# Advaith-Sajeev/LiDAR-Vision-VQA

Hardware: AMD Instinct MI355X
Metric: fused tokens/sec/GPU + cross-attn MFMA-roofline % (32k pts x 196 patches) (higher is better)
Workload: dtype bf16; 1 GPU; BASELINE configs[1]: 32768-pt scenes (Dist-C) -> hard voxelise (0.1, 0.1, 0.2) T=10 max=60000 + MeanVFE; pillars (0.2, 0.2, 8.0) T=20 max=30000 -> PillarVFE[64] -> PointPillarScatter 512x512 (as an index map; sparse key stream: K|V computed only for the cells with a pillar in their 3x3 neighbourhood, by LayerNorm and the K|V projection folded onto the 64-channel conv token, every other key from th; parallelism=scene-parallel x1

## Files before the change

### lidar-vision-vqa_amd/csrc/bev_tiles.hip

```cpp
#include "common.h"
#include <type_traits>
#include <utility>

namespace bt {

typedef __attribute__((ext_vector_type(8))) short bf16x8;
typedef __attribute__((ext_vector_type(4))) float f32x4;
typedef __attribute__((ext_vector_type(2))) __bf16 bf16x2_t;
typedef uint32_t u32x4 __attribute__((ext_vector_type(4)));

__device__ __forceinline__ uint32_t pack_bf16(float a, float b) {
    bf16x2_t p = {(__bf16)a, (__bf16)b};
    return *reinterpret_cast<uint32_t *>(&p);
}
typedef _Float16 f16x2_t __attribute__((ext_vector_type(2)));
__device__ __forceinline__ uint32_t pack_f16(float a, float b) {
    f16x2_t p = {(_Float16)a, (_Float16)b};
    return __builtin_bit_cast(uint32_t, p);
}

constexpr int TS = 8, TCELLS = 64;
constexpr int NPIECE = 8, PCELLS = 8;
constexpr int PH = 4, PW = 6, PHALO = PH * PW;
constexpr int NSLOT = NPIECE * PHALO;
// ... 832 lines not shown
    __syncthreads();
    if (g_begin >= g_end) return;
    {
        int c0, c1;
        const int i0 = load_idx(g_begin, c0);
        const int i1 = g_begin + g_step < g_end ? load_idx(g_begin + g_step, c1) : (c1 = -1, -1);
        store_idx(idxh, i0, c0);
        store_idx(idxh + 256, i1, c1);
    }
    __syncthreads();
    dma_halo(idxh);
    asm volatile("s_waitcnt vmcnt(0)" ::: "memory");
    __syncthreads();
    conv_tile(idxh, 0);
    int buf = 0;
    for (int64_t g = g_begin, it = 0; g < g_end; g += g_step, ++it) {
        __syncthreads();
        const int32_t *ih_cur = idxh + (it & 1) * 256, *ih_nx = idxh + ((it + 1) & 1) * 256;
        const bool has_nx = g + g_step < g_end, has_n2 = g + 2 * g_step < g_end;
        if (has_nx) dma_halo(ih_nx);
        int code_cur[4];
#pragma unroll
        for (int gq = 0; gq < 4; ++gq) code_cur[gq] = ih_cur[200 + 2 * gq + (l15 >> 3)];
        int c2 = -1;
        const int i2 = has_n2 ? load_idx(g + 2 * g_step, c2) : -1;
        {
            const int rt = wid & 3;
            const uint16_t *rp = r_hi + (16 * rt + l15) * C + 8 * g4, *rpl = r_lo + (16 * rt + l15) * C + 8 * g4;
            const bf16x8 ra0 = *reinterpret_cast<const bf16x8 *>(rp), ra1 = *reinterpret_cast<const bf16x8 *>(rp + 32);
            bf16x8 rl0 = ra0, rl1 = ra1;
            if (X3) { rl0 = *reinterpret_cast<const bf16x8 *>(rpl); rl1 = *reinterpret_cast<const bf16x8 *>(rpl + 32); }
            const f32x4 rinit = *reinterpret_cast<const f32x4 *>(r0s + 16 * rt + 4 * g4);
#pragma unroll
            for (int u = 0; u < 2; ++u) {
                const int gq = 2 * (wid >> 2) + u;
                bf16x8 th0, th1, tl0, tl1;
                load_t(buf, gq, th0, th1, tl0, tl1);
                f32x4 v = rinit;
                v = __builtin_amdgcn_mfma_f32_16x16x32_bf16(ra0, th0, v, 0, 0, 0);
                v = __builtin_amdgcn_mfma_f32_16x16x32_bf16(ra1, th1, v, 0, 0, 0);
                if (X3) {
                    v = __builtin_amdgcn_mfma_f32_16x16x32_bf16(ra0, tl0, v, 0, 0, 0);
                    v = __builtin_amdgcn_mfma_f32_16x16x32_bf16(ra1, tl1, v, 0, 0, 0);
                    v = __builtin_amdgcn_mfma_f32_16x16x32_bf16(rl0, th0, v, 0, 0, 0);
                    v = __builtin_amdgcn_mfma_f32_16x16x32_bf16(rl1, th1, v, 0, 0, 0);
                }
                float sq = (v[0] * v[0] + v[1] * v[1]) + (v[2] * v[2] + v[3] * v[3]);
                sq += __shfl_xor(sq, 16);
                sq += __shfl_xor(sq, 32);
                if (g4 == 0) part[(buf * 4 + rt) * TCELLS + gq * 16 + l15] = sq;
            }
        }
        asm volatile("s_waitcnt vmcnt(0)" ::: "memory");
        __syncthreads();
        store_idx(idxh + (it & 1) * 256, i2, c2);
        {
            const float *pr = part + buf * 4 * TCELLS;
            auto cell_of = [&](int gq) { return gq * 16 + l15; };
            auto code_of = [&](int gq) { return gq == 0 ? code_cur[0] : gq == 1 ? code_cur[1] : gq == 2 ? code_cur[2] : code_cur[3]; };
            auto request = [&](int gq, f32x4 (&te)[2 * JH], int2 &pd) {
                const int cell = cell_of(gq), code = code_of(gq);
                const bool in_list = code >= 0;
                const int64_t prow = in_list ? (int64_t)((code >> 3) / a.S) * TCELLS + (code & 7) * PCELLS + (cell & 7) : 0;
                pd = in_list ? a.piece_dirty[g * NPIECE + (cell >> 3)] : make_int2(0, 0);
                const float *tep = a.te + prow * (2 * N) + ncol0 + col0;
#pragma unroll
                for (int jj = 0; jj < 2 * JH; ++jj) te[jj] = *reinterpret_cast<const f32x4 *>(tep + 4 * jj);
            };
            auto emit = [&](int gq, const f32x4 (&te)[2 * JH], const int2 pd) {
                const int cell = cell_of(gq);
                const bool valid = (pd.y >> (cell & 7)) & 1;
                const int64_t orow = pd.x + __popc((unsigned)pd.y & ((1u << (cell & 7)) - 1u));
                const float ss = (pr[cell] + pr[TCELLS + cell]) + (pr[2 * TCELLS + cell] + pr[3 * TCELLS + cell]) + a.c0;
                const float rstd = 1.0f / sqrtf(ss * a.inv_d + a.eps);
                bf16x8 th0, th1, tl0, tl1;
                load_t(buf, gq, th0, th1, tl0, tl1);
                uint16_t *dst = a.out + orow * (2 * N) + ncol0 + col0;
                auto half_out = [&](auto hf_tag) {
                    constexpr int HF = decltype(hf_tag)::value;
                    f32x4 acc[JH];
                    product(hf_tag, th0, th1, tl0, tl1, acc);
                    uint32_t oh[2 * JH];
#pragma unroll
                    for (int jj = 0; jj < JH; ++jj) {
                        const f32x4 tv = te[HF * JH + jj];
                        oh[2 * jj] = pack_bf16(acc[jj][0] * rstd + tv[0], acc[jj][1] * rstd + tv[1]);
                        oh[2 * jj + 1] = pack_bf16(acc[jj][2] * rstd + tv[2], acc[jj][3] * rstd + tv[3]);
                    }
                    if (valid) {
#pragma unroll
                        for (int q = 0; q < 2 * JH; q += 2)
                            *reinterpret_cast<uint2 *>(dst + 2 * (2 * HF * JH + q)) = make_uint2(oh[q], oh[q + 1]);
                    }
                };
                half_out(std::integral_constant<int, 0>{});
                half_out(std::integral_constant<int, 1>{});
            };
            f32x4 te_a[2 * JH], te_b[2 * JH];
            int2 pd_a, pd_b;
            request(0, te_a, pd_a);
            if (has_nx) conv_tile(ih_nx, buf ^ 1);
            request(1, te_b, pd_b);
            emit(0, te_a, pd_a);
            request(2, te_a, pd_a);
            emit(1, te_b, pd_b);
            request(3, te_b, pd_b);
            emit(2, te_a, pd_a);
            emit(3, te_b, pd_b);
        }
        buf ^= 1;
    }
}

struct ConvArgs {
    const float *feat;
    const int32_t *idx;
    const int32_t *live_list;
    const int2 *piece_dirty;
    const int32_t *counts;
    const float *w9, *b9;
    const uint16_t *rh, *rl;
    const float *r0;
    float c0, inv_d, eps;
    int S, H, W;
    uint16_t *th, *tl;
    float *rstd;
    int32_t *key;
};

typedef int i32x2 __attribute__((ext_vector_type(2)));
template <int N> __device__ __forceinline__ void vm_wait() { asm volatile("s_waitcnt vmcnt(%0)" ::"n"(N) : "memory"); }
template <int OFF> __device__ __forceinline__ void vm_load16(f32x4 &d, const void *p) {
    asm volatile("global_load_dwordx4 %0, %1, off offset:%2" : "=&v"(d) : "v"(p), "n"(OFF) : "memory");
}
__device__ __forceinline__ void vm_load8(i32x2 &d, const void *p) { asm volatile("global_load_dwordx2 %0, %1, off" : "=&v"(d) : "v"(p) : "memory"); }
template <class T> __device__ __forceinline__ void vm_load4(T &d, const void *p) {
    static_assert(sizeof(T) == 4, "one dword");
    asm volatile("global_load_dword %0, %1, off" : "=&v"(d) : "v"(p) : "memory");
}
__device__ __forceinline__ void vm_dma16(const void *src, uint32_t dst) {
    uint32_t keep;
    asm volatile("s_mov_b32 %0, m0\n\ts_mov_b32 m0, %2\n\ts_nop 0\n\tglobal_load_lds_dwordx4 %1, off\n\ts_mov_b32 m0, %0"
                 : "=&s"(keep) : "v"(src), "s"(dst) : "memory");
}
template <class T> __device__ __forceinline__ void landed(T &x) { asm volatile("" : "+v"(x)); }
template <int... I, class F> __device__ __forceinline__ void static_for(std::integer_sequence<int, I...>, F &&f) { (f(std::integral_constant<int, I>{}), ...); }
template <int N, class F> __device__ __forceinline__ void static_for(F &&f) { static_for(std::make_integer_sequence<int, N>{}, f); }
__device__ __forceinline__ void lds_barrier() {
    asm volatile("s_waitcnt lgkmcnt(0)" ::: "memory");
    __builtin_amdgcn_s_barrier();
    asm volatile("" ::: "memory");
}

template <bool X3>
__global__ void __launch_bounds__(512) k_conv_rows(ConvArgs a) {
    constexpr int C = 64, NWV = 8, RING = 8;
    extern __shared__ __attribute__((aligned(16))) uint8_t smem[];
    uint16_t *t_hi = reinterpret_cast<uint16_t *>(smem);
    uint16_t *t_lo = t_hi + TCELLS * C;
    float *halo = reinterpret_cast<float *>(t_lo + TCELLS * C);
    int32_t *idxh = reinterpret_cast<int32_t *>(halo + 2 * NSLOT * C);
    int32_t *mcode = idxh + 2 * 256;
    i32x2 *mdirty = reinterpret_cast<i32x2 *>(mcode + RING * NPIECE);
    float *part = reinterpret_cast<float *>(mdirty + RING * NPIECE);
    const int tid = threadIdx.x, lane = tid & 63, wid = tid >> 6, l15 = lane & 15, g4 = lane >> 4;
    const int tw = a.W / TS;
    const int n_live = a.counts[0];
    const int64_t n_groups = ((int64_t)n_live + NPIECE - 1) / NPIECE;
    const int64_t g_begin = blockIdx.x, g_step = gridDim.x;
    if (g_begin >= n_groups) return;
    const int n_my = (int)((n_groups - g_begin + g_step - 1) / g_step);

    float wk[9][8], bk[8];
#pragma unroll
    for (int c = 0; c < 8; ++c) {
        const int ch = (tid & 7) * 8 + c;
        bk[c] = a.b9 ? a.b9[ch] : 0.f;
#pragma unroll
        for (int k = 0; k < 9; ++k) wk[k][c] = a.w9[ch * 9 + k];
    }
    const int rt = wid & 3;
    bf16x8 ra0, ra1, rl0, rl1;
    {
        const uint16_t *rp = a.rh + (16 * rt + l15) * C + 8 * g4;
        ra0 = *reinterpret_cast<const bf16x8 *>(rp);
        ra1 = *reinterpret_cast<const bf16x8 *>(rp + 32);
        rl0 = ra0; rl1 = ra1;
        if (X3) {
            const uint16_t *rpl = a.rl + (16 * rt + l15) * C + 8 * g4;
            rl0 = *reinterpret_cast<const bf16x8 *>(rpl);
            rl1 = *reinterpret_cast<const bf16x8 *>(rpl + 32);
        }
    }
    f32x4 rinit = *reinterpret_cast<const f32x4 *>(a.r0 + 16 * rt + 4 * g4);

    auto piece_k = [&](int o, int j, bool &ok) -> int64_t {
        const int64_t grp = g_begin + (int64_t)o * g_step, k = grp * NPIECE + j;
        ok = o < n_my && k < n_live;
        return ok ? k : 0;
    };
    auto idx_off = [&](int o, bool &ok) -> int64_t {
        ok = false;
        if (tid >= NSLOT) return 0;
        const int j = tid / PHALO, hc = tid - j * PHALO;
        const int code = mcode[(o & (RING - 1)) * NPIECE + j];
        if (code < 0) return 0;
        const int p = code & 7, ts = code >> 3, t = ts / a.S, sc = ts - t * a.S;
        int y0, x0;
        piece_origin(t, p, tw, y0, x0);
        const int gy = y0 - 1 + hc / PW, gx = x0 - 1 + hc % PW;
        if (gy < 0 || gy >= a.H || gx < 0 || gx >= a.W) return 0;
        ok = true;
        return ((int64_t)sc * a.H + gy) * a.W + gx;
    };
    const uint32_t lds_halo = (uint32_t)(uintptr_t)((__attribute__((address_space(3))) float *)halo);
    auto dma_halo = [&](const int32_t *ih, int hbuf) {
        for (int q = wid; q < NSLOT / 4; q += NWV) {
            const int row = ih[q * 4 + (lane >> 4)];
            const uint32_t dst = __builtin_amdgcn_readfirstlane(lds_halo + (uint32_t)((hbuf * NSLOT + q * 4) * C * 4));
            if (row >= 0) vm_dma16(a.feat + (int64_t)row * C + 4 * l15, dst);
        }
    };
    auto conv_tile = [&](const int32_t *ih, const float *hl, int o) {
        const int cell = tid >> 3, cg = (tid & 7) * 8, hb = (cell >> 3) * PHALO, cy = (cell >> 2) & 1, cx = cell & 3;
        float acc[8];
#pragma unroll
        for (int c = 0; c < 8; ++c) acc[c] = bk[c];
#pragma unroll
        for (int rr = 0; rr < 3; ++rr)
#pragma unroll
            for (int k = 0; k < 3; ++k) {
                const int slot = hb + (cy + rr) * PW + cx + k;
                if (ih[slot] >= 0) {
                    const f32x4 v0 = *reinterpret_cast<const f32x4 *>(hl + slot * C + cg), v1 = *reinterpret_cast<const f32x4 *>(hl + slot * C + cg + 4);
                    const float *kk = wk[rr * 3 + k];
#pragma unroll
                    for (int c = 0; c < 4; ++c) { acc[c] = fmaf(v0[c], kk[c], acc[c]); acc[4 + c] = fmaf(v1[c], kk[4 + c], acc[4 + c]); }
                }
            }
        uint32_t hi[4], lo[4];
#pragma unroll
        for (int c = 0; c < 4; ++c) {
            const float y0 = gelu_erf(acc[2 * c]), y1 = gelu_erf(acc[2 * c + 1]);
            hi[c] = pack_bf16(y0, y1);
            lo[c] = pack_bf16(y0 - __uint_as_float(hi[c] << 16), y1 - __uint_as_float(hi[c] & 0xffff0000u));
        }
        const int ch = (tid & 7) ^ ((cell >> 1) & 7);
        *reinterpret_cast<u32x4 *>(t_hi + cell * C + ch * 8) = u32x4{hi[0], hi[1], hi[2], hi[3]};
        if (X3) *reinterpret_cast<u32x4 *>(t_lo + cell * C + ch * 8) = u32x4{lo[0], lo[1], lo[2], lo[3]};
        const int m = (o & (RING - 1)) * NPIECE + (cell >> 3);
        if (mcode[m] >= 0) {
            const i32x2 pd = mdirty[m];
            if ((pd.y >> (cell & 7)) & 1) {
                const int64_t orow = pd.x + __popc((unsigned)pd.y & ((1u << (cell & 7)) - 1u));
                *reinterpret_cast<u32x4 *>(a.th + orow * C + cg) = u32x4{hi[0], hi[1], hi[2], hi[3]};
                if (X3) *reinterpret_cast<u32x4 *>(a.tl + orow * C + cg) = u32x4{lo[0], lo[1], lo[2], lo[3]};
            }
        }
    };
    auto row_sums = [&]() {
#pragma unroll
        for (int u = 0; u < 2; ++u) {
            const int gq = 2 * (wid >> 2) + u;
            const int row = gq * 16 + l15;
            const int c0 = (g4 ^ ((row >> 1) & 7)) * 8, c1 = ((4 + g4) ^ ((row >> 1) & 7)) * 8;
            const bf16x8 th0 = *reinterpret_cast<const bf16x8 *>(t_hi + row * C + c0), th1 = *reinterpret_cast<const bf16x8 *>(t_hi + row * C + c1);
            f32x4 v = rinit;
            v = __builtin_amdgcn_mfma_f32_16x16x32_bf16(ra0, th0, v, 0, 0, 0);
            v = __builtin_amdgcn_mfma_f32_16x16x32_bf16(ra1, th1, v, 0, 0, 0);
            if (X3) {
                const bf16x8 tl0 = *reinterpret_cast<const bf16x8 *>(t_lo + row * C + c0), tl1 = *reinterpret_cast<const bf16x8 *>(t_lo + row * C + c1);
                v = __builtin_amdgcn_mfma_f32_16x16x32_bf16(ra0, tl0, v, 0, 0, 0);
                v = __builtin_amdgcn_mfma_f32_16x16x32_bf16(ra1, tl1, v, 0, 0, 0);
                v = __builtin_amdgcn_mfma_f32_16x16x32_bf16(rl0, th0, v, 0, 0, 0);
                v = __builtin_amdgcn_mfma_f32_16x16x32_bf16(rl1, th1, v, 0, 0, 0);
            }
            float sq = (v[0] * v[0] + v[1] * v[1]) + (v[2] * v[2] + v[3] * v[3]);
            sq += __shfl_xor(sq, 16);
            sq += __shfl_xor(sq, 32);
            if (g4 == 0) part[rt * TCELLS + gq * 16 + l15] = sq;
        }
    };
    auto finish_rows = [&](int o) {
        if (wid != NWV - 1) return;
        const int cell = lane, m = (o & (RING - 1)) * NPIECE + (cell >> 3);
        const int code = mcode[m];
        if (code < 0) return;
        const i32x2 pd = mdirty[m];
        if ((pd.y >> (cell & 7)) & 1) {
            const int64_t orow = pd.x + __popc((unsigned)pd.y & ((1u << (cell & 7)) - 1u));
            const float ss = (part[cell] + part[TCELLS + cell]) + (part[2 * TCELLS + cell] + part[3 * TCELLS + cell]) + a.c0;
            a.rstd[orow] = 1.0f / sqrtf(ss * a.inv_d + a.eps);
            a.key[orow] = ((code >> 3) / a.S) * TCELLS + (code & 7) * PCELLS + (cell & 7);
        }
    };

    if (tid < 4 * NPIECE) {
        bool ok;
        const int64_t k = piece_k(tid >> 3, tid & 7, ok);
        const int code = a.live_list[k];
        const int2 pd = a.piece_dirty[k];
        mcode[tid] = ok ? code : -1;
        mdirty[tid] = ok ? i32x2{pd.x, pd.y} : i32x2{0, 0};
    }
    __syncthreads();
    {
        bool k0, k1, k2;
        const int64_t o0 = idx_off(0, k0), o1 = idx_off(1, k1), o2 = idx_off(2, k2);
        const int i0 = a.idx[o0], i1 = a.idx[o1], i2 = a.idx[o2];
        if (tid < 256) { idxh[tid] = k0 ? i0 : -1; idxh[256 + tid] = k1 ? i1 : -1; }
        __syncthreads();
        dma_halo(idxh, 0);
        dma_halo(idxh + 256, 1);
        vm_wait<0>();
        landed(ra0); landed(ra1); landed(rl0); landed(rl1); landed(rinit);
#pragma unroll
        for (int c = 0; c < 8; ++c) {
            landed(bk[c]);
#pragma unroll
            for (int k = 0; k < 9; ++k) landed(wk[k][c]);
        }
        __syncthreads();
        conv_tile(idxh, halo, 0);
        __syncthreads();
        row_sums();
        if (tid < 256) idxh[tid] = k2 ? i2 : -1;
        __syncthreads();
    }
    for (int it = 0; it < n_my; ++it) {
        const int cur = it & 1, nx = cur ^ 1;
        const bool has_nx = it + 1 < n_my;
        dma_halo(idxh + cur * 256, cur);
        bool ok_i, ok_m;
        const int64_t off_i = idx_off(it + 3, ok_i);
        const int64_t k_m = piece_k(it + 4, tid & 7, ok_m);
        int iw, mc;
        i32x2 md;
        vm_load4(iw, a.idx + off_i);
        vm_load4(mc, a.live_list + k_m);
        vm_load8(md, a.piece_dirty + k_m);
        finish_rows(it);
        if (has_nx) conv_tile(idxh + nx * 256, halo + nx * NSLOT * C, it + 1);
        lds_barrier();
        if (has_nx) row_sums();
        vm_wait<0>();
        landed(iw); landed(mc); landed(md);
        if (tid < 256) idxh[nx * 256 + tid] = ok_i ? iw : -1;
        if (tid < NPIECE) {
            const int m = ((it + 4) & (RING - 1)) * NPIECE + tid;
            mcode[m] = ok_m ? mc : -1;
            mdirty[m] = ok_m ? md : i32x2{0, 0};
        }
        lds_barrier();
    }
}

struct KvRowArgs {
    const uint16_t *th, *tl;
    const float *rstd;
    const int32_t *key;
    const int32_t *n_rows;
    const uint16_t *mh, *ml;
    const float *m0;
    const float *te;
    uint16_t *out;
    int k_fp16;
};

template <int J, bool X3, bool TH>
__global__ void __launch_bounds__(512) k_kv_rows(KvRowArgs a) {
    constexpr int N = 128 * J, C = 64, JH = J / 2;
    static_assert(J % 2 == 0, "even J");
    extern __shared__ __attribute__((aligned(16))) uint8_t smem[];
    uint16_t *t_hi = reinterpret_cast<uint16_t *>(smem);
    uint16_t *t_lo = t_hi + 2 * TCELLS * C;
    float *pbias = reinterpret_cast<float *>(t_lo + 2 * TCELLS * C);
    constexpr int SROW = N + 8;
    uint16_t *sbuf = reinterpret_cast<uint16_t *>(pbias + N);
    const int tid = threadIdx.x, lane = tid & 63, wid = tid >> 6, l15 = lane & 15, g4 = lane >> 4;
    const int64_t n_rows = *a.n_rows;
    const int64_t n_groups = (n_rows + TCELLS - 1) / TCELLS;
    const bool x8 = gridDim.x >= 16 && gridDim.x % 16 == 0;
    const int nxcd = x8 ? 8 : 1;
    const int xcd = x8 ? (int)blockIdx.x & 7 : 0;
    const int half = x8 ? ((int)blockIdx.x >> 3) & 1 : (int)blockIdx.x & 1;
    const int wg_r = x8 ? (int)blockIdx.x >> 4 : (int)blockIdx.x >> 1, wg_R = x8 ? (int)gridDim.x >> 4 : ((int)gridDim.x + 1) >> 1;
    const int64_t per_x = (n_groups + nxcd - 1) / nxcd;
    const int64_t x_begin = (int64_t)xcd * per_x, x_end = x_begin + per_x < n_groups ? x_begin + per_x : n_groups;
    const int64_t g_begin = x_begin + wg_r, g_end = x_end, g_step = wg_R;
    const int ncol0 = half * N;
    const bool as_f16 = a.k_fp16 != 0 && half == 0;
    for (int e = tid; e < N; e += 512) pbias[e] = a.m0[ncol0 + e];

    bf16x8 wf[J][2], wfl[X3 ? J : 1][2];
#pragma unroll
    for (int j = 0; j < J; ++j) {
        const int n = ncol0 + 16 * J * wid + (TH ? 32 * (j >> 1) + 8 * (l15 >> 2) + 4 * (j & 1) + (l15 & 3) : 16 * j + l15);
        wf[j][0] = *reinterpret_cast<const bf16x8 *>(a.mh + (int64_t)n * C + 8 * g4);
        wf[j][1] = *reinterpret_cast<const bf16x8 *>(a.mh + (int64_t)n * C + 32 + 8 * g4);
        if (X3) {
            wfl[j][0] = *reinterpret_cast<const bf16x8 *>(a.ml + (int64_t)n * C + 8 * g4);
            wfl[j][1] = *reinterpret_cast<const bf16x8 *>(a.ml + (int64_t)n * C + 32 + 8 * g4);
        }
    }
    const int col0 = 16 * J * wid + (TH ? 8 : 4) * g4;
    auto colj = [&](int j) { return TH ? 32 * (j >> 1) + 4 * (j & 1) : 16 * j; };
    const uint32_t lds_t = (uint32_t)(uintptr_t)((__attribute__((address_space(3))) uint16_t *)t_hi);
    auto stage = [&](int64_t g, int buf) {
        const int row = 8 * wid + (lane >> 3), c = lane & 7;
        int64_t r = g * TCELLS + row;
        r = r < n_rows ? r : n_rows - 1;
        const int64_t so = r * C + ((c ^ ((row >> 1) & 7)) << 3);
        const uint32_t dst = __builtin_amdgcn_readfirstlane(lds_t + (uint32_t)((buf * TCELLS + 8 * wid) * C * 2));
        vm_dma16(a.th + so, dst);
        if (X3) vm_dma16(a.tl + so, dst + 2 * TCELLS * C * 2);
    };
    auto load_t = [&](int buf, int gq, bf16x8 &th0, bf16x8 &th1, bf16x8 &tl0, bf16x8 &tl1) {
        const int row = gq * 16 + l15;
        const int c0 = (g4 ^ ((row >> 1) & 7)) * 8, c1 = ((4 + g4) ^ ((row >> 1) & 7)) * 8;
        th0 = *reinterpret_cast<const bf16x8 *>(t_hi + (buf * TCELLS + row) * C + c0);
        th1 = *reinterpret_cast<const bf16x8 *>(t_hi + (buf * TCELLS + row) * C + c1);
        if (X3) {
            tl0 = *reinterpret_cast<const bf16x8 *>(t_lo + (buf * TCELLS + row) * C + c0);
            tl1 = *reinterpret_cast<const bf16x8 *>(t_lo + (buf * TCELLS + row) * C + c1);
        }
    };
    const uint32_t lds_bias = (uint32_t)(uintptr_t)((__attribute__((address_space(3))) float *)pbias) + 4 * col0;
    auto product = [&](auto hf_tag, const bf16x8 &th0, const bf16x8 &th1, const bf16x8 &tl0, const bf16x8 &tl1, f32x4 (&acc)[JH]) {
        constexpr int HF = decltype(hf_tag)::value;
        uint32_t pb = lds_bias;
        asm volatile("" : "+v"(pb));
#pragma unroll
        for (int jj = 0; jj < JH; ++jj) {
            const int j = HF * JH + jj;
            acc[jj] = *(const __attribute__((address_space(3))) f32x4 *)(pb + 4 * colj(j));
            acc[jj] = __builtin_amdgcn_mfma_f32_16x16x32_bf16(wf[j][0], th0, acc[jj], 0, 0, 0);
            acc[jj] = __builtin_amdgcn_mfma_f32_16x16x32_bf16(wf[j][1], th1, acc[jj], 0, 0, 0);
            if (X3) {
                acc[jj] = __builtin_amdgcn_mfma_f32_16x16x32_bf16(wf[j][0], tl0, acc[jj], 0, 0, 0);
                acc[jj] = __builtin_amdgcn_mfma_f32_16x16x32_bf16(wf[j][1], tl1, acc[jj], 0, 0, 0);
                acc[jj] = __builtin_amdgcn_mfma_f32_16x16x32_bf16(wfl[j][0], th0, acc[jj], 0, 0, 0);
                acc[jj] = __builtin_amdgcn_mfma_f32_16x16x32_bf16(wfl[j][1], th1, acc[jj], 0, 0, 0);
            }
        }
    };
    if (g_begin >= g_end) return;
    constexpr int R = TH ? JH : J;
    constexpr int S = N / 256;
    constexpr int D = X3 ? 2 : 1;
    constexpr int M = 8;
#pragma unroll
    for (int j = 0; j < J; ++j) {
        landed(wf[j][0]);
        landed(wf[j][1]);
        if (X3) { landed(wfl[j][0]); landed(wfl[j][1]); }
    }
    auto load_meta = [&](int64_t g, int (&kq)[4], float (&rq)[4]) {
#pragma unroll
        for (int q = 0; q < 4; ++q) {
            int64_t r = g * TCELLS + q * 16 + l15;
            r = r < n_rows ? r : n_rows - 1;
            vm_load4(kq[q], a.key + r);
            vm_load4(rq[q], a.rstd + r);
        }
    };
    auto meta_landed = [&](int (&kq)[4], float (&rq)[4]) {
#pragma unroll
        for (int q = 0; q < 4; ++q) { landed(kq[q]); landed(rq[q]); }
    };
    auto request = [&](int key, f32x4 (&te)[R]) {
        const char *tep = TH ? reinterpret_cast<const char *>(reinterpret_cast<const uint16_t *>(a.te) + (int64_t)key * (2 * N) + ncol0 + col0)
                             : reinterpret_cast<const char *>(a.te + (int64_t)key * (2 * N) + ncol0 + col0);
        static_for<R>([&](auto i) { vm_load16<64 * decltype(i)::value>(te[decltype(i)::value], tep); });
    };
    int kq[4], kn[4];
    float rq[4], rn[4];
    f32x4 te_a[R], te_b[R];
    load_meta(g_begin, kq, rq);
    stage(g_begin, 0);
    vm_wait<D>();
    meta_landed(kq, rq);
    request(kq[0], te_a);
    vm_wait<R>();
    int buf = 0;
    for (int64_t g = g_begin; g < g_end; g += g_step) {
        const bool first = g == g_begin, full = (g + 1) * TCELLS <= n_rows;
        asm volatile("s_waitcnt lgkmcnt(0)" ::: "memory");
        __builtin_amdgcn_s_barrier();
        asm volatile("" ::: "memory");
        const int64_t gn = g + g_step < g_end ? g + g_step : g;
        stage(gn, buf ^ 1);
        load_meta(gn, kn, rn);
        auto emit = [&](int gq, f32x4 (&te)[R], auto &&wait) {
            bf16x8 th0, th1, tl0, tl1;
            load_t(buf, gq, th0, th1, tl0, tl1);
            const float rs = gq == 0 ? rq[0] : gq == 1 ? rq[1] : gq == 2 ? rq[2] : rq[3];
            uint16_t *sb = sbuf + (gq & 1) * 16 * SROW;
            uint16_t *dst = sb + l15 * SROW + col0;
            auto half_out = [&](auto hf_tag) {
                constexpr int HF = decltype(hf_tag)::value;
                f32x4 acc[JH];
                product(hf_tag, th0, th1, tl0, tl1, acc);
                if constexpr (HF == 0) {
                    wait();
#pragma unroll
                    for (int i = 0; i < R; ++i) landed(te[i]);
// ... 10 lines not shown
                    } else {
                        tv = te[TH ? 0 : j];
                    }
                    if (as_f16) {
                        oh[2 * jj] = pack_f16(acc[jj][0] * rs + tv[0], acc[jj][1] * rs + tv[1]);
                        oh[2 * jj + 1] = pack_f16(acc[jj][2] * rs + tv[2], acc[jj][3] * rs + tv[3]);
                    } else {
                        oh[2 * jj] = pack_bf16(acc[jj][0] * rs + tv[0], acc[jj][1] * rs + tv[1]);
                        oh[2 * jj + 1] = pack_bf16(acc[jj][2] * rs + tv[2], acc[jj][3] * rs + tv[3]);
                    }
                }
#pragma unroll
                for (int jj = 0; jj < JH; ++jj)
                    *reinterpret_cast<uint2 *>(dst + colj(HF * JH + jj)) = make_uint2(oh[2 * jj], oh[2 * jj + 1]);
            };
            half_out(std::integral_constant<int, 0>{});
            half_out(std::integral_constant<int, 1>{});
            asm volatile("s_waitcnt lgkmcnt(0)" ::: "memory");
            __builtin_amdgcn_s_barrier();
            asm volatile("" ::: "memory");
            constexpr int UPR = N / 8;
#pragma unroll
            for (int i = 0; i < S; ++i) {
                const int u = (wid * S + i) * 64 + lane, row = u / UPR, c16 = u - row * UPR;
                const int64_t r = g * TCELLS + gq * 16 + row;
                if (r < n_rows)
                    *reinterpret_cast<u32x4 *>(a.out + r * (2 * N) + ncol0 + c16 * 8) = *reinterpret_cast<const u32x4 *>(sb + row * SROW + c16 * 8);
            }
        };
        auto wait_sr = [&]() { if (full) vm_wait<S + R>(); else vm_wait<R>(); };
        request(kq[1], te_b);
        emit(0, te_a, [&]() {
            if (first) vm_wait<D + M + R>(); else vm_wait<S + D + M + R>();
        });
        request(kq[2], te_a);
        emit(1, te_b, [&]() {
            wait_sr();
            meta_landed(kn, rn);
        });
        request(kq[3], te_b);
        emit(2, te_a, [&]() { wait_sr(); });
        request(kn[0], te_a);
        emit(3, te_b, [&]() { wait_sr(); });
#pragma unroll
        for (int q = 0; q < 4; ++q) { kq[q] = kn[q]; rq[q] = rn[q]; }
        buf ^= 1;
    }
    vm_wait<0>();
}

}

extern "C" size_t lvq_bev_tiles_workspace_bytes(int batch, int ny, int nx) {
    if (batch <= 0 || ny <= 0 || nx <= 0) return 0;
    const int64_t total = (int64_t)batch * (ny / 8) * (nx / 8) * bt::NPIECE;
    return lvq_align((size_t)2 * lvq_cdiv(total, bt::CNT_BLOCK) * sizeof(int32_t)) + lvq_align((size_t)total) + 512;
}

extern "C" int lvq_bev_tiles(const int32_t *idx_map, int batch, int ny, int nx, int force_all, int row_base, int32_t *live_list,
                             int32_t *piece_dirty, int32_t *row_src, int32_t *counts, void *ws, size_t ws_bytes, lvq_stream_t stream) {
    if (batch <= 0 || ny <= 0 || nx <= 0 || row_base < 0 || !live_list || !piece_dirty || !row_src || !counts || (!idx_map && !force_all)) return LVQ_EINVAL;
    if ((ny % bt::TS) || (nx % bt::TS)) return LVQ_EUNSUPPORTED;
    const int64_t total = (int64_t)batch * (ny / bt::TS) * (nx / bt::TS) * bt::NPIECE;
    if ((int64_t)row_base + total * bt::PCELLS > 0x7fffffff || batch > 65535) return LVQ_EUNSUPPORTED;
    if (((uintptr_t)row_src & 15) || ((uintptr_t)piece_dirty & 7) || ((uintptr_t)idx_map & 15)) return LVQ_EUNSUPPORTED;
    const int nb = (int)((total + bt::CNT_BLOCK - 1) / bt::CNT_BLOCK);
    LvqArena arena(ws, ws_bytes);
    int32_t *block_cnt = arena.take<int32_t>((size_t)2 * nb);
    uint8_t *masks = arena.take<uint8_t>((size_t)total);
    if (!arena.ok) return LVQ_EWORKSPACE;
    hipStream_t st = lvq_s(stream);
    hipLaunchKernelGGL(bt::k_piece_count, dim3(nb), dim3(256), 0, st, idx_map, batch, ny, nx, force_all, total, block_cnt, masks);
    hipLaunchKernelGGL(bt::k_piece_compact, dim3(nb), dim3(256), 0, st, idx_map, batch, ny, nx, force_all, total, (const int32_t *)block_cnt,
                       (const uint8_t *)masks, nb, row_base, live_list, reinterpret_cast<int2 *>(piece_dirty), row_src, counts);
    return lvq_launch_status();
}

template <int J> static int launch_tile_kv(const bt::KvArgs &a, bool x3, int64_t cap_tiles, hipStream_t st) {
    const size_t lds = (size_t)2 * 2 * bt::TCELLS * 64 * 2 + (size_t)bt::NSLOT * 64 * 4 + 2 * 256 * 4 + (size_t)2 * 4 * bt::TCELLS * 4 +
                       (size_t)128 * J * 4 + 9 * 64 * 4 + 64 * 4 + 64 * 4 + (size_t)2 * 64 * 64 * 2;
    static LvqLdsOnce once;
    if (!lvq_ensure_lds(once, {(const void *)bt::k_tile_kv<J, false>, (const void *)bt::k_tile_kv<J, true>}, lds)) return LVQ_ELAUNCH;
    int64_t grid = (int64_t)lvq_cu_count();
    if (grid > cap_tiles) grid = cap_tiles;
    grid *= 2;
    if (x3) hipLaunchKernelGGL((bt::k_tile_kv<J, true>), dim3((unsigned)grid), dim3(512), lds, st, a);
    else    hipLaunchKernelGGL((bt::k_tile_kv<J, false>), dim3((unsigned)grid), dim3(512), lds, st, a);
    return lvq_launch_status();
}

template <int J> static int launch_kv_rows(const bt::KvRowArgs &a, bool x3, bool t_f16, int64_t cap_tiles, hipStream_t st) {
    const size_t lds = (size_t)2 * 2 * bt::TCELLS * 64 * 2 + (size_t)128 * J * 4 + (size_t)2 * 16 * (128 * J + 8) * 2;
    static LvqLdsOnce once;
    if (lds > 64 * 1024 && !lvq_ensure_lds(once, {(const void *)bt::k_kv_rows<J, false, false>, (const void *)bt::k_kv_rows<J, true, false>,
                                                   (const void *)bt::k_kv_rows<J, false, true>, (const void *)bt::k_kv_rows<J, true, true>}, lds))
        return LVQ_ELAUNCH;
    int64_t grid = (int64_t)lvq_cu_count();
    if (grid > cap_tiles) grid = cap_tiles;
    grid *= 2;
    if (t_f16) {
        if (x3) hipLaunchKernelGGL((bt::k_kv_rows<J, true, true>), dim3((unsigned)grid), dim3(512), lds, st, a);
        else    hipLaunchKernelGGL((bt::k_kv_rows<J, false, true>), dim3((unsigned)grid), dim3(512), lds, st, a);
    } else {
        if (x3) hipLaunchKernelGGL((bt::k_kv_rows<J, true, false>), dim3((unsigned)grid), dim3(512), lds, st, a);
        else    hipLaunchKernelGGL((bt::k_kv_rows<J, false, false>), dim3((unsigned)grid), dim3(512), lds, st, a);
    }
    return lvq_launch_status();
}

extern "C" size_t lvq_bev_tile_kv_workspace_bytes(int64_t cap_tiles) {
    if (cap_tiles <= 0) return 0;
    LvqSizer z;
    z.take<uint16_t>((size_t)cap_tiles * 64 * 64);
    z.take<uint16_t>((size_t)cap_tiles * 64 * 64);
    z.take<float>((size_t)cap_tiles * 64);
    z.take<int32_t>((size_t)cap_tiles * 64);
    return z.total();
}

extern "C" int lvq_bev_tile_kv(const float *pillar_feat, const int32_t *idx_map, const int32_t *live_list, const int32_t *piece_dirty,
                               const int32_t *counts, int64_t cap_tiles, int batch, int ny, int nx, int c_in, const float *w9, const float *b9,
                               const lvq_bf16 *m, const lvq_bf16 *m_lo, const float *m0, const lvq_bf16 *r, const lvq_bf16 *r_lo, const float *r0,
                               float c0, int d_ln, float eps, const void *t_tiled, int t_f16, int n, int k_fp16, lvq_bf16 *kv, void *ws,
                               size_t ws_bytes, lvq_stream_t stream) {
    if (batch <= 0 || ny <= 0 || nx <= 0 || cap_tiles <= 0 || d_ln <= 0 || !idx_map || !live_list || !piece_dirty || !counts || !w9 || !m || !m0 || !r ||
        !r0 || !t_tiled || !kv)
        return LVQ_EINVAL;
    if ((m_lo == nullptr) != (r_lo == nullptr)) return LVQ_EINVAL;
    if ((k_fp16 || t_f16) && ws == nullptr) return LVQ_EUNSUPPORTED;
    if (c_in != 64 || (ny % 8) || (nx % 8) || (n % 256) || n < 256 || n > 1024) return LVQ_EUNSUPPORTED;
    if (((uintptr_t)pillar_feat | (uintptr_t)m | (uintptr_t)m_lo | (uintptr_t)r | (uintptr_t)r_lo | (uintptr_t)m0 | (uintptr_t)r0 | (uintptr_t)t_tiled |
         (uintptr_t)kv) & 15)
        return LVQ_EUNSUPPORTED;
    bt::KvArgs a;
    a.feat = pillar_feat; a.idx = idx_map; a.live_list = live_list; a.piece_dirty = reinterpret_cast<const int2 *>(piece_dirty); a.counts = counts;
    a.w9 = w9; a.b9 = b9; a.mh = m; a.ml = m_lo; a.m0 = m0; a.rh = r; a.rl = r_lo; a.r0 = r0; a.c0 = c0; a.inv_d = 1.0f / (float)d_ln; a.eps = eps;
    a.te = static_cast<const float *>(t_tiled); a.S = batch; a.H = ny; a.W = nx; a.out = kv;
    hipStream_t st = lvq_s(stream);
    const bool x3 = m_lo != nullptr;
    if (ws != nullptr) {
        LvqArena arena(ws, ws_bytes);
        uint16_t *th = arena.take<uint16_t>((size_t)cap_tiles * 64 * 64);
        uint16_t *tl = arena.take<uint16_t>((size_t)cap_tiles * 64 * 64);
        float *rstd = arena.take<float>((size_t)cap_tiles * 64);
        int32_t *key = arena.take<int32_t>((size_t)cap_tiles * 64);
        if (!arena.ok) return LVQ_EWORKSPACE;
        bt::ConvArgs c;
        c.feat = pillar_feat; c.idx = idx_map; c.live_list = live_list; c.piece_dirty = a.piece_dirty; c.counts = counts; c.w9 = w9; c.b9 = b9;
        c.rh = r; c.rl = r_lo; c.r0 = r0; c.c0 = c0; c.inv_d = a.inv_d; c.eps = eps; c.S = batch; c.H = ny; c.W = nx;
        c.th = th; c.tl = x3 ? tl : nullptr; c.rstd = rstd; c.key = key;
        const size_t lds = (size_t)2 * bt::TCELLS * 64 * 2 + (size_t)2 * bt::NSLOT * 64 * 4 + 2 * 256 * 4 + (size_t)8 * bt::NPIECE * (4 + 8) +
                           (size_t)4 * bt::TCELLS * 4;
        static LvqLdsOnce once;
        if (!lvq_ensure_lds(once, {(const void *)bt::k_conv_rows<false>, (const void *)bt::k_conv_rows<true>}, lds)) return LVQ_ELAUNCH;
        int64_t grid = (int64_t)lvq_cu_count();
        const int hook = lvq_tune().conv_rows_grid;
        if (hook > 0) grid = hook < grid ? hook : grid;
        else if (grid > cap_tiles) grid = cap_tiles;
        if (x3) hipLaunchKernelGGL((bt::k_conv_rows<true>), dim3((unsigned)grid), dim3(512), lds, st, c);
        else    hipLaunchKernelGGL((bt::k_conv_rows<false>), dim3((unsigned)grid), dim3(512), lds, st, c);
        bt::KvRowArgs k;
        k.th = th; k.tl = x3 ? tl : nullptr; k.rstd = rstd; k.key = key; k.n_rows = counts + 2; k.mh = m; k.ml = m_lo; k.m0 = m0; k.te = static_cast<const float *>(t_tiled); k.out = kv; k.k_fp16 = k_fp16;
        switch (n / 128) {
            case 2: return launch_kv_rows<2>(k, x3, t_f16 != 0, cap_tiles, st);
            case 4: return launch_kv_rows<4>(k, x3, t_f16 != 0, cap_tiles, st);
            case 6: return launch_kv_rows<6>(k, x3, t_f16 != 0, cap_tiles, st);
            case 8: return launch_kv_rows<8>(k, x3, t_f16 != 0, cap_tiles, st);
            default: return LVQ_EUNSUPPORTED;
        }
    }
    switch (n / 128) {
        case 2: return launch_tile_kv<2>(a, x3, cap_tiles, st);
        case 4: return launch_tile_kv<4>(a, x3, cap_tiles, st);
        case 6: return launch_tile_kv<6>(a, x3, cap_tiles, st);
        case 8: return launch_tile_kv<8>(a, x3, cap_tiles, st);
        default: return LVQ_EUNSUPPORTED;
    }
}

extern "C" int lvq_bev_scene_pairs(const int32_t *row_src, int batch, int n_tiles, int row_base, int cap_tiles, int32_t *pair_src,
                                   int32_t *pair_info, lvq_stream_t stream) {
    if (!row_src || !pair_src || !pair_info || batch <= 0 || n_tiles <= 0 || cap_tiles <= 0 || row_base < 0) return LVQ_EINVAL;
    if (((uintptr_t)row_src & 15) || (int64_t)n_tiles * bt::TCELLS > 0x7fffffff || batch > 65535) return LVQ_EUNSUPPORTED;
    if (cap_tiles >= n_tiles && cap_tiles >= 2 && !lvq_tune().pairs_one_wg) {
        const int64_t ne = (int64_t)n_tiles * bt::TCELLS;
        int64_t chunk = (ne + 63) / 64;
        chunk = (chunk + 1023) / 1024 * 1024;
        const int nch = (int)((ne + chunk - 1) / chunk);
        hipLaunchKernelGGL(bt::k_scene_pair_count, dim3(nch, batch), dim3(bt::PAIR2_NT), 0, lvq_s(stream), row_src, n_tiles, row_base, cap_tiles, (int)chunk,
                           pair_src);
        hipLaunchKernelGGL(bt::k_scene_pair_write, dim3(nch, batch), dim3(bt::PAIR2_NT), 0, lvq_s(stream), row_src, n_tiles, row_base, cap_tiles, (int)chunk,
                           nch, pair_src, pair_info);
        return lvq_launch_status();
    }
    hipLaunchKernelGGL(bt::k_scene_pairs, dim3(batch), dim3(bt::PAIR_NT), 0, lvq_s(stream), row_src, n_tiles, row_base, cap_tiles, pair_src, pair_info);
    return lvq_launch_status();
}

extern "C" int lvq_bev_shared_lists(const int32_t *row_src, int batch, int n_tiles, int row_base, int cap_tiles, int32_t *list_src, int32_t *list_info,
                                    void *ws, size_t ws_bytes, lvq_stream_t stream) {
    if (!row_src || !list_src || !list_info || batch <= 0 || n_tiles <= 0 || cap_tiles <= 0 || row_base < 0) return LVQ_EINVAL;
    if (((uintptr_t)row_src & 15) || (int64_t)n_tiles * bt::TCELLS > 0x7fffffff || batch > 65534) return LVQ_EUNSUPPORTED;
    if (cap_tiles < n_tiles) return LVQ_EUNSUPPORTED;
    const int ne = n_tiles * bt::TCELLS;
    LvqArena arena(ws, ws_bytes);
    uint8_t *flag = arena.take<uint8_t>((size_t)ne);
    int32_t *cnt = arena.take<int32_t>((size_t)(2 * batch + 1) * 64);
    if (!arena.ok) return LVQ_EWORKSPACE;
    int64_t chunk = ((int64_t)ne + 63) / 64;
    chunk = (chunk + 1023) / 1024 * 1024;
    const int nch = (int)(((int64_t)ne + chunk - 1) / chunk);
    hipStream_t st = lvq_s(stream);
    hipLaunchKernelGGL(bt::k_shared_flags, dim3((unsigned)lvq_cdiv(ne, bt::SH_NT * 4)), dim3(bt::SH_NT), 0, st, row_src, batch, ne, row_base, flag);
    hipLaunchKernelGGL(bt::k_shared_count, dim3(nch, batch), dim3(bt::SH_NT), 0, st, row_src, flag, batch, n_tiles, row_base, (int)chunk, cnt);
    hipLaunchKernelGGL(bt::k_shared_write, dim3(nch, batch + 1), dim3(bt::SH_NT), 0, st, row_src, flag, batch, n_tiles, row_base, cap_tiles, (int)chunk,
                       nch, cnt, list_src, list_info);
    return lvq_launch_status();
}

template <int J> static int launch_tile_tokens(const bt::TokArgs &a, bool x3, bool olo, int64_t cap_tiles, hipStream_t st) {
    const size_t lds = (size_t)2 * 2 * bt::TCELLS * 64 * 2 + (size_t)bt::NSLOT * 64 * 4 + 2 * 256 * 4 + (size_t)2 * 8 * bt::TCELLS * 2 * 4 +
                       (size_t)3 * 128 * J * 4 + 9 * 64 * 4 + 64 * 4;
    static LvqLdsOnce once;
    if (!lvq_ensure_lds(once, {(const void *)bt::k_tile_tokens<J, false, false>, (const void *)bt::k_tile_tokens<J, true, false>,
                               (const void *)bt::k_tile_tokens<J, true, true>}, lds))
        return LVQ_ELAUNCH;
    int64_t grid = (int64_t)lvq_cu_count();
    if (grid > cap_tiles) grid = cap_tiles;
    if (x3 && olo) hipLaunchKernelGGL((bt::k_tile_tokens<J, true, true>), dim3((unsigned)grid), dim3(512), lds, st, a);
    else if (x3)   hipLaunchKernelGGL((bt::k_tile_tokens<J, true, false>), dim3((unsigned)grid), dim3(512), lds, st, a);
    else           hipLaunchKernelGGL((bt::k_tile_tokens<J, false, false>), dim3((unsigned)grid), dim3(512), lds, st, a);
    return lvq_launch_status();
}

extern "C" int lvq_bev_tile_tokens(const float *pillar_feat, const int32_t *idx_map, const int32_t *live_list, const int32_t *piece_dirty,
                                   const int32_t *counts, int64_t cap_tiles, int batch, int ny, int nx, int c_in, const float *w9, const float *b9, const lvq_bf16 *w,
                                   const lvq_bf16 *w_lo, const float *bias, const float *gamma, const float *beta, float eps, const float *pe_tiled,
                                   int n, lvq_bf16 *x, lvq_bf16 *x_lo, lvq_stream_t stream) {
    if (batch <= 0 || ny <= 0 || nx <= 0 || cap_tiles <= 0 || !idx_map || !live_list || !piece_dirty || !counts || !w9 || !w || !gamma || !pe_tiled || !x)
        return LVQ_EINVAL;
    if (x_lo && !w_lo) return LVQ_EINVAL;
    if (c_in != 64 || (ny % 8) || (nx % 8) || (n % 256) || n < 256 || n > 1024) return LVQ_EUNSUPPORTED;
    if (((uintptr_t)pillar_feat | (uintptr_t)w | (uintptr_t)w_lo | (uintptr_t)pe_tiled | (uintptr_t)x | (uintptr_t)x_lo | (uintptr_t)bias |
         (uintptr_t)gamma | (uintptr_t)beta) & 15)
        return LVQ_EUNSUPPORTED;
    bt::TokArgs a;
    a.feat = pillar_feat; a.idx = idx_map; a.live_list = live_list; a.piece_dirty = reinterpret_cast<const int2 *>(piece_dirty); a.counts = counts; a.w9 = w9; a.b9 = b9; a.wh = w; a.wl = w_lo;
    a.bias = bias; a.gamma = gamma; a.beta = beta; a.pe = pe_tiled; a.eps = eps; a.S = batch; a.H = ny; a.W = nx; a.xh = x; a.xl = x_lo;
    hipStream_t st = lvq_s(stream);
    const bool x3 = w_lo != nullptr, olo = x_lo != nullptr;
    switch (n / 128) {
        case 2: return launch_tile_tokens<2>(a, x3, olo, cap_tiles, st);
        case 4: return launch_tile_tokens<4>(a, x3, olo, cap_tiles, st);
        case 6: return launch_tile_tokens<6>(a, x3, olo, cap_tiles, st);
        case 8: return launch_tile_tokens<8>(a, x3, olo, cap_tiles, st);
        default: return LVQ_EUNSUPPORTED;
    }
}
```

Before: 1.147 million fused tokens/s.

## Compact dirty cells per group so depthwise conv runs only on live cells

```diff
diff --git a/lidar-vision-vqa_amd/csrc/bev_tiles.hip b/lidar-vision-vqa_amd/csrc/bev_tiles.hip
--- a/lidar-vision-vqa_amd/csrc/bev_tiles.hip
+++ b/lidar-vision-vqa_amd/csrc/bev_tiles.hip
@@ -1008,9 +1008,14 @@
     asm volatile("" ::: "memory");
 }
 
-template <bool X3>
+#ifndef LVQ_CONV_TASK_CELLS
+#define LVQ_CONV_TASK_CELLS 4
+#endif
+constexpr int CONV_TASK_CELLS = LVQ_CONV_TASK_CELLS;
+template <bool X3, int CP>
 __global__ void __launch_bounds__(512) k_conv_rows(ConvArgs a) {
-    constexpr int C = 64, NWV = 8, RING = 8;
+    static_assert(CP == 1 || CP == 2 || CP == 4 || CP == 8, "cells per task = channels per lane");
+    constexpr int C = 64, NWV = 8, RING = 8, LPC = 64 / CP;
     extern __shared__ __attribute__((aligned(16))) uint8_t smem[];
     uint16_t *t_hi = reinterpret_cast<uint16_t *>(smem);
     uint16_t *t_lo = t_hi + TCELLS * C;
@@ -1027,10 +1032,12 @@
     if (g_begin >= n_groups) return;
     const int n_my = (int)((n_groups - g_begin + g_step - 1) / g_step);
 
-    float wk[9][8], bk[8];
-#pragma unroll
-    for (int c = 0; c < 8; ++c) {
-        const int ch = (tid & 7) * 8 + c;
+    const int wv = __builtin_amdgcn_readfirstlane(wid);
+    const int cg = (lane & (LPC - 1)) * CP;
+    float wk[9][CP], bk[CP];
+#pragma unroll
+    for (int c = 0; c < CP; ++c) {
+        const int ch = cg + c;
         bk[c] = a.b9 ? a.b9[ch] : 0.f;
 #pragma unroll
         for (int k = 0; k < 9; ++k) wk[k][c] = a.w9[ch * 9 + k];
@@ -1077,47 +1084,117 @@
             if (row >= 0) vm_dma16(a.feat + (int64_t)row * C + 4 * l15, dst);
         }
     };
-    auto conv_tile = [&](const int32_t *ih, const float *hl, int o) {
-        const int cell = tid >> 3, cg = (tid & 7) * 8, hb = (cell >> 3) * PHALO, cy = (cell >> 2) & 1, cx = cell & 3;
-        float acc[8];
-#pragma unroll
-        for (int c = 0; c < 8; ++c) acc[c] = bk[c];
-#pragma unroll
-        for (int rr = 0; rr < 3; ++rr)
-#pragma unroll
-            for (int k = 0; k < 3; ++k) {
-                const int slot = hb + (cy + rr) * PW + cx + k;
-                if (ih[slot] >= 0) {
-                    const f32x4 v0 = *reinterpret_cast<const f32x4 *>(hl + slot * C + cg), v1 = *reinterpret_cast<const f32x4 *>(hl + slot * C + cg + 4);
-                    const float *kk = wk[rr * 3 + k];
-#pragma unroll
-                    for (int c = 0; c < 4; ++c) { acc[c] = fmaf(v0[c], kk[c], acc[c]); acc[4 + c] = fmaf(v1[c], kk[4 + c], acc[4 + c]); }
+    constexpr int NT = CP > 1 ? NWV / CP : 1;
+    struct GroupRank { int n, first, cell, tc[NT]; };
+    auto rank_load = [&](int o) -> i32x2 { return mdirty[(o & (RING - 1)) * NPIECE + (lane >> 3)]; };
+    auto rank_finish = [&](const i32x2 &e) -> GroupRank {
+        const bool dirty = ((e.y >> (lane & 7)) & 1) != 0;
+        const uint64_t M = __ballot(dirty);
+        GroupRank g;
+        g.n = __popcll(M);
+        g.first = __builtin_amdgcn_readlane(e.x, M ? __ffsll((long long)M) - 1 : 0);
+        const int rk = __builtin_amdgcn_mbcnt_hi((uint32_t)(M >> 32), __builtin_amdgcn_mbcnt_lo((uint32_t)M, 0));
+        g.cell = __builtin_amdgcn_ds_permute((dirty ? rk : g.n + lane - rk) * 4, lane);
+#pragma unroll
+        for (int i = 0; i < NT; ++i) g.tc[i] = CP > 1 ? __shfl(g.cell, (wv + NWV * i) * CP + lane / LPC) : 0;
+        return g;
+    };
+    auto conv_tile = [&](const int32_t *ih, const float *hl, const GroupRank &g) {
+        auto window = [](int cell) { return (cell >> 3) * PHALO + ((cell >> 2) & 1) * PW + (cell & 3); };
+        if constexpr (CP == 1) {
+            auto fetch = [&](int r, int &iw, float (&v)[9]) {
+                const int hb = window(__builtin_amdgcn_readlane(g.cell, r));
+                const int kk = lane < 9 ? lane : 0;
+                iw = ih[hb + (kk / 3) * PW + kk % 3];
+                const float *hp = hl + hb * C + lane;
+#pragma unroll
+                for (int k = 0; k < 9; ++k) v[k] = hp[((k / 3) * PW + k % 3) * C];
+            };
+            if (wv >= g.n) return;
+            int iw;
+            float v[9];
+            fetch(wv, iw, v);
+#pragma unroll 2
+            for (int r = wv; r < g.n; r += NWV) {
+                const int rn = r + NWV < g.n ? r + NWV : r;
+                int iw_n;
+                float v_n[9];
+                fetch(rn, iw_n, v_n);
+                const unsigned live = (unsigned)__ballot(lane < 9 && iw >= 0);
+                float acc = bk[0];
+#pragma unroll
+                for (int k = 0; k < 9; ++k)
+                    if ((live >> k) & 1u) acc = fmaf(v[k], wk[k][0], acc);
+                const float y = gelu_erf(acc);
+                const uint32_t hi = pack_bf16(y, 0.f);
+                const int at = r * C + (((lane >> 3) ^ ((r >> 1) & 7)) * 8) + (lane & 7);
+                t_hi[at] = (uint16_t)hi;
+                if (X3) t_lo[at] = (uint16_t)pack_bf16(y - __uint_as_float(hi << 16), 0.f);
+                iw = iw_n;
+#pragma unroll
+                for (int k = 0; k < 9; ++k) v[k] = v_n[k];
+            }
+        } else {
+            typedef float fvec __attribute__((ext_vector_type(CP)));
+            int iw[NT][9];
+            fvec v[NT][9];
+#pragma unroll
+            for (int i = 0; i < NT; ++i)
+                if ((wv + NWV * i) * CP < g.n) {
+                    const int hb = window(g.tc[i]);
+#pragma unroll
+                    for (int k = 0; k < 9; ++k) iw[i][k] = ih[hb + (k / 3) * PW + k % 3];
+#pragma unroll
+                    for (int k = 0; k < 9; ++k) v[i][k] = *reinterpret_cast<const fvec *>(hl + (hb + (k / 3) * PW + k % 3) * C + cg);
+                }
+#pragma unroll
+            for (int i = 0; i < NT; ++i) {
+                const int r = (wv + NWV * i) * CP + lane / LPC;
+                if ((wv + NWV * i) * CP < g.n && r < g.n) {
+                    float acc[CP];
+#pragma unroll
+                    for (int c = 0; c < CP; ++c) acc[c] = bk[c];
+#pragma unroll
+                    for (int k = 0; k < 9; ++k)
+                        if (iw[i][k] >= 0) {
+                            asm volatile("");
+#pragma unroll
+                            for (int c = 0; c < CP; ++c) acc[c] = fmaf(v[i][k][c], wk[k][c], acc[c]);
+                        }
+                    uint32_t *ph = reinterpret_cast<uint32_t *>(t_hi + r * C + (((cg >> 3) ^ ((r >> 1) & 7)) * 8) + (cg & 7));
+                    uint32_t *pl = reinterpret_cast<uint32_t *>(t_lo + r * C + (((cg >> 3) ^ ((r >> 1) & 7)) * 8) + (cg & 7));
+#pragma unroll
+                    for (int c = 0; c < CP / 2; ++c) {
+                        const float y0 = gelu_erf(acc[2 * c]), y1 = gelu_erf(acc[2 * c + 1]);
+                        const uint32_t hi = pack_bf16(y0, y1);
+                        ph[c] = hi;
+                        if (X3) pl[c] = pack_bf16(y0 - __uint_as_float(hi << 16), y1 - __uint_as_float(hi & 0xffff0000u));
+                    }
                 }
             }
-        uint32_t hi[4], lo[4];
-#pragma unroll
-        for (int c = 0; c < 4; ++c) {
-            const float y0 = gelu_erf(acc[2 * c]), y1 = gelu_erf(acc[2 * c + 1]);
-            hi[c] = pack_bf16(y0, y1);
-            lo[c] = pack_bf16(y0 - __uint_as_float(hi[c] << 16), y1 - __uint_as_float(hi[c] & 0xffff0000u));
-        }
-        const int ch = (tid & 7) ^ ((cell >> 1) & 7);
-        *reinterpret_cast<u32x4 *>(t_hi + cell * C + ch * 8) = u32x4{hi[0], hi[1], hi[2], hi[3]};
-        if (X3) *reinterpret_cast<u32x4 *>(t_lo + cell * C + ch * 8) = u32x4{lo[0], lo[1], lo[2], lo[3]};
-        const int m = (o & (RING - 1)) * NPIECE + (cell >> 3);
-        if (mcode[m] >= 0) {
-            const i32x2 pd = mdirty[m];
-            if ((pd.y >> (cell & 7)) & 1) {
-                const int64_t orow = pd.x + __popc((unsigned)pd.y & ((1u << (cell & 7)) - 1u));
-                *reinterpret_cast<u32x4 *>(a.th + orow * C + cg) = u32x4{hi[0], hi[1], hi[2], hi[3]};
-                if (X3) *reinterpret_cast<u32x4 *>(a.tl + orow * C + cg) = u32x4{lo[0], lo[1], lo[2], lo[3]};
-            }
-        }
-    };
-    auto row_sums = [&]() {
+        }
+    };
+    auto take_t = [&](const GroupRank &g, u32x4 &h, u32x4 &l) {
+        const int row = tid >> 3, c8 = tid & 7;
+        if (row < g.n) {
+            const int at = row * C + ((c8 ^ ((row >> 1) & 7)) * 8);
+            h = *reinterpret_cast<const u32x4 *>(t_hi + at);
+            if (X3) l = *reinterpret_cast<const u32x4 *>(t_lo + at);
+        }
+    };
+    auto put_t = [&](const GroupRank &g, const u32x4 &h, const u32x4 &l) {
+        const int row = tid >> 3, c8 = tid & 7;
+        if (row < g.n) {
+            const int64_t orow = (int64_t)g.first + row;
+            *reinterpret_cast<u32x4 *>(a.th + orow * C + c8 * 8) = h;
+            if (X3) *reinterpret_cast<u32x4 *>(a.tl + orow * C + c8 * 8) = l;
+        }
+    };
+    auto row_sums = [&](int n) {
 #pragma unroll
         for (int u = 0; u < 2; ++u) {
-            const int gq = 2 * (wid >> 2) + u;
+            const int gq = (wv >> 2) + 2 * u;
+            if (gq * 16 >= n) continue;
             const int row = gq * 16 + l15;
             const int c0 = (g4 ^ ((row >> 1) & 7)) * 8, c1 = ((4 + g4) ^ ((row >> 1) & 7)) * 8;
             const bf16x8 th0 = *reinterpret_cast<const bf16x8 *>(t_hi + row * C + c0), th1 = *reinterpret_cast<const bf16x8 *>(t_hi + row * C + c1);
@@ -1137,20 +1214,19 @@
             if (g4 == 0) part[rt * TCELLS + gq * 16 + l15] = sq;
         }
     };
-    auto finish_rows = [&](int o) {
-        if (wid != NWV - 1) return;
-        const int cell = lane, m = (o & (RING - 1)) * NPIECE + (cell >> 3);
-        const int code = mcode[m];
-        if (code < 0) return;
-        const i32x2 pd = mdirty[m];
-        if ((pd.y >> (cell & 7)) & 1) {
-            const int64_t orow = pd.x + __popc((unsigned)pd.y & ((1u << (cell & 7)) - 1u));
-            const float ss = (part[cell] + part[TCELLS + cell]) + (part[2 * TCELLS + cell] + part[3 * TCELLS + cell]) + a.c0;
+    auto finish_rows = [&](int o, const GroupRank &g) {
+        if (wv != NWV - 1) return;
+        if (lane < g.n) {
+            const int code = mcode[(o & (RING - 1)) * NPIECE + (g.cell >> 3)];
+            const int64_t orow = (int64_t)g.first + lane;
+            const float ss = (part[lane] + part[TCELLS + lane]) + (part[2 * TCELLS + lane] + part[3 * TCELLS + lane]) + a.c0;
             a.rstd[orow] = 1.0f / sqrtf(ss * a.inv_d + a.eps);
-            a.key[orow] = ((code >> 3) / a.S) * TCELLS + (code & 7) * PCELLS + (cell & 7);
-        }
-    };
-
+            a.key[orow] = ((code >> 3) / a.S) * TCELLS + (code & 7) * PCELLS + (g.cell & 7);
+        }
+    };
+
+    u32x4 sh{}, sl{};
+    GroupRank gc, g;
     if (tid < 4 * NPIECE) {
         bool ok;
         const int64_t k = piece_k(tid >> 3, tid & 7, ok);
@@ -1171,15 +1247,18 @@
         vm_wait<0>();
         landed(ra0); landed(ra1); landed(rl0); landed(rl1); landed(rinit);
 #pragma unroll
-        for (int c = 0; c < 8; ++c) {
+        for (int c = 0; c < CP; ++c) {
             landed(bk[c]);
 #pragma unroll
             for (int k = 0; k < 9; ++k) landed(wk[k][c]);
         }
         __syncthreads();
-        conv_tile(idxh, halo, 0);
+        gc = rank_finish(rank_load(0));
+        g = rank_finish(rank_load(1));
+        conv_tile(idxh, halo, gc);
         __syncthreads();
-        row_sums();
+        take_t(gc, sh, sl);
+        row_sums(gc.n);
         if (tid < 256) idxh[tid] = k2 ? i2 : -1;
         __syncthreads();
     }
@@ -1195,10 +1274,16 @@
         vm_load4(iw, a.idx + off_i);
         vm_load4(mc, a.live_list + k_m);
         vm_load8(md, a.piece_dirty + k_m);
-        finish_rows(it);
-        if (has_nx) conv_tile(idxh + nx * 256, halo + nx * NSLOT * C, it + 1);
+        const i32x2 e2 = rank_load(it + 2);
+        put_t(gc, sh, sl);
+        finish_rows(it, gc);
+        if (has_nx) conv_tile(idxh + nx * 256, halo + nx * NSLOT * C, g);
+        const GroupRank gn = rank_finish(e2);
         lds_barrier();
-        if (has_nx) row_sums();
+        if (has_nx) {
+            take_t(g, sh, sl);
+            row_sums(g.n);
+        }
         vm_wait<0>();
         landed(iw); landed(mc); landed(md);
         if (tid < 256) idxh[nx * 256 + tid] = ok_i ? iw : -1;
@@ -1208,6 +1293,8 @@
             mdirty[m] = ok_m ? md : i32x2{0, 0};
         }
         lds_barrier();
+        gc = g;
+        g = gn;
     }
 }
 
@@ -1524,13 +1611,14 @@
         const size_t lds = (size_t)2 * bt::TCELLS * 64 * 2 + (size_t)2 * bt::NSLOT * 64 * 4 + 2 * 256 * 4 + (size_t)8 * bt::NPIECE * (4 + 8) +
                            (size_t)4 * bt::TCELLS * 4;
         static LvqLdsOnce once;
-        if (!lvq_ensure_lds(once, {(const void *)bt::k_conv_rows<false>, (const void *)bt::k_conv_rows<true>}, lds)) return LVQ_ELAUNCH;
+        constexpr int CP = bt::CONV_TASK_CELLS;
+        if (!lvq_ensure_lds(once, {(const void *)bt::k_conv_rows<false, CP>, (const void *)bt::k_conv_rows<true, CP>}, lds)) return LVQ_ELAUNCH;
         int64_t grid = (int64_t)lvq_cu_count();
         const int hook = lvq_tune().conv_rows_grid;
         if (hook > 0) grid = hook < grid ? hook : grid;
         else if (grid > cap_tiles) grid = cap_tiles;
-        if (x3) hipLaunchKernelGGL((bt::k_conv_rows<true>), dim3((unsigned)grid), dim3(512), lds, st, c);
-        else    hipLaunchKernelGGL((bt::k_conv_rows<false>), dim3((unsigned)grid), dim3(512), lds, st, c);
+        if (x3) hipLaunchKernelGGL((bt::k_conv_rows<true, CP>), dim3((unsigned)grid), dim3(512), lds, st, c);
+        else    hipLaunchKernelGGL((bt::k_conv_rows<false, CP>), dim3((unsigned)grid), dim3(512), lds, st, c);
         bt::KvRowArgs k;
         k.th = th; k.tl = x3 ? tl : nullptr; k.rstd = rstd; k.key = key; k.n_rows = counts + 2; k.mh = m; k.ml = m_lo; k.m0 = m0; k.te = static_cast<const float *>(t_tiled); k.out = kv; k.k_fp16 = k_fp16;
         switch (n / 128) {
```

Measured after the change: 1.145 million fused tokens/s. Within noise of the previous version (-0.1%).
